# yumingj/C2-Matching

Measured on AMD Instinct MI355X. Metric: LR-Ref image pairs/sec (160x160 LR, 500x500 Ref, 4x SR), higher is better.
Workload: dtype f32

## Files before the change

### c2-matching_amd/c2m_amd/ops.py

```python
import torch

from . import _lib


def _dev_f32(t, name):
    if not isinstance(t, torch.Tensor) or not t.is_cuda:
        raise _lib.C2MError(f"{name} must be a tensor on the GPU (the HIP path has no CPU fallback)")
    if t.dtype != torch.float32:
        raise _lib.C2MError(f"{name} must be float32, got {t.dtype}")
    return t if t.is_contiguous() else t.contiguous()


def _stream():
    return torch.cuda.current_stream().cuda_stream


def _pair(v):
    return (int(v), int(v)) if isinstance(v, int) else (int(v[0]), int(v[1]))


class NormalizedFeatures(torch.Tensor):

    @staticmethod
    def wrap(t, ss):
# ... 589 lines not shown


def _wino4_ok(srcs, weight, out_mode, W):
    return _WINO4 and W % 64 == 0 and out_mode == "nhwc" and _wino_ok(srcs, weight, out_mode, W)


def bf16_autocast():
    return torch.is_autocast_enabled('cuda') and torch.get_autocast_dtype('cuda') == torch.bfloat16


def _split_ok(srcs, weight, fast):
    return ((_SPLIT == "all" or (fast and _SPLIT != "0")) and all(s.shape[1] % 16 == 0 for s in srcs) and
            sum(s.shape[1] for s in srcs) == weight.shape[1])


def conv3x3(srcs, weight, bias=None, act=ACT_NONE, slope=0.1, res1=None, res2=None, out_mode="nhwc", out=None, algo=None,
            out2_grouped8=None, fast=False, out_dtype=None, dword_stores=False):
    srcs = list(srcs) if isinstance(srcs, (list, tuple)) else [srcs]
    B, _, H, W = srcs[0].shape
    Cin = sum(s.shape[1] for s in srcs)
    Cout = weight.shape[0]
    dev = srcs[0].device
    if algo is None:
        reduced = bf16_autocast()
        if (out2_grouped8 is None and (_split_ok(srcs, weight, fast) or (reduced and _split_ok(srcs, weight, True))) and (out_mode != "nhwc_pool2" or (H % 2 == 0 and W % 2 == 0))
                and (out_mode not in ("nhwc", "nhwc_pool2") or Cout % 4 == 0)):
            kind = 4 if reduced else 6 if _f16x2_auto() else 3
        else:
            kind = 2 if (fast and _wino4_ok(srcs, weight, out_mode, W)) else 1 if _wino_ok(srcs, weight, out_mode, W) else 0
    elif algo in ALGO_IDS:
        kind = ALGO_IDS[algo]
    else:
        raise _lib.C2MError(f"conv3x3: unknown algo {algo!r} (one of {', '.join(ALGO_IDS)})")
# ... 15 lines not shown
    if out is not None:
        out_dtype = out.dtype
    if out_dtype == torch.bfloat16:
        io |= 2
    elif out_dtype not in (None, torch.float32):
        raise _lib.C2MError("conv3x3: out_dtype is float32 or bfloat16")
    for bit, r in ((4, res1), (8, res2)):
        if r is not None and r.dtype == torch.bfloat16:
            io |= bit
    if io and (kind != 4 or out_mode != "nhwc"):
        raise _lib.C2MError("conv3x3: bfloat16 tensors need the bf16 kernel (algo='bf16' / bf16 autocast) in nhwc mode")
    if dword_stores:
        if io or kind not in (3, 4, 6) or out_mode not in ("pixel_shuffle", "nchw"):
            raise _lib.C2MError("conv3x3: dword_stores selects a store path of the split kernels' pixel_shuffle / nchw epilogues")
        io = 16
    d.io_flags = io
    d.wr = wr.data_ptr()
    if bias is not None:
        bias = _dev_f32(bias.detach(), "bias")
    d.bias = bias.data_ptr() if bias is not None else None
    d.act, d.slope = int(act), float(slope)
    if out_mode == "nhwc":
        if out is None:
            out = empty_nhwc(B, Cout, H, W, dev, torch.bfloat16 if io & 2 else torch.float32)
        d.out_mode = 0
        o = _nhwc_src(out, "out", bf16_ok=True)
        d.out_pix_pitch, d.out_row_pitch, d.out_img_pitch = o.pix_pitch, o.row_pitch, o.img_pitch
        for name, r in (("res1", res1), ("res2", res2)):
            if r is not None:
                rs = _nhwc_src(r, name, bf16_ok=True)
# ... 15 lines not shown
        o = _nhwc_src(out, "out")
        d.out_pix_pitch, d.out_row_pitch, d.out_img_pitch = o.pix_pitch, o.row_pitch, o.img_pitch
    elif out_mode == "nchw":
        out = torch.empty((B, Cout, H, W), dtype=torch.float32, device=dev)
        d.out_mode = 2
    else:
        raise _lib.C2MError(f"unknown out_mode {out_mode}")
    d.out = out.data_ptr()
    if kind == 6:
        d.range_flag = _range_flag(dev).data_ptr()
    with torch.cuda.device(dev):
        _lib.check(_lib.lib().c2m_conv3x3_nhwc_f32(_stream(), d), "c2m_conv3x3_nhwc_f32")
    if _ConvFlops.enabled:
        f = 2.0 * Cout * 9 * Cin * H * W * B
        _ConvFlops.add(_KINDS[kind].family, f, f * _KINDS[kind].exec_factor)
    return out


def conv3x3_dgrad(grad_out, weight):
    Cout, Cin = weight.shape[:2]
    B, Cg, H, W = grad_out.shape
    if Cg != Cout or Cout % 16 != 0 or Cin % 4 != 0:
        raise _lib.C2MError("conv3x3_dgrad: grad_out channels must equal weight.shape[0] (a multiple of 16); Cin % 4 == 0")
    wr = _wcache.get(weight, kind=5)
    out = empty_nhwc(B, Cin, H, W, grad_out.device)
    d = _lib.Conv3x3Desc()
    d.algo = _KINDS[5].algo
    d.B, d.H, d.W, d.Cin, d.Cout, d.nsrc = B, H, W, Cout, Cin, 1
    d.src[0] = _nhwc_src(grad_out, "grad_out")
    d.wr = wr.data_ptr()
    d.out_mode = 0
# ... 127 lines not shown


def index_to_flow(max_idx):
    if not max_idx.is_cuda or max_idx.dtype != torch.int64 or max_idx.dim() != 3:
        raise _lib.C2MError("max_idx must be an int64 GPU tensor [B, hq, wq]")
    mi = max_idx.contiguous()
    B, hq, wq = mi.shape
    flow = torch.empty((B, hq, wq, 2), dtype=torch.float32, device=mi.device)
    with torch.cuda.device(mi.device):
        _lib.check(_lib.lib().c2m_index_to_flow_f32(_stream(), mi.data_ptr(), B, hq, wq, flow.data_ptr()), "c2m_index_to_flow_f32")
    return flow


def conv3x3_dcn_head(srcs, weight, bias, deformable_groups, flow=None, scale=1, abs_sum=None, algo=None):
    srcs = list(srcs) if isinstance(srcs, (list, tuple)) else [srcs]
    B, _, H, W = srcs[0].shape
    Cin = sum(s.shape[1] for s in srcs)
    dg = int(deformable_groups)
    Cout = weight.shape[0]
    if Cout != 3 * dg * 9:
        raise _lib.C2MError("conv3x3_dcn_head: weight must have 3*dg*9 output channels")
    dev = srcs[0].device
    bias = _dev_f32(bias.detach(), "bias")
    offset = torch.empty((B, 2 * dg * 9, H, W), dtype=torch.float32, device=dev)
    mask = torch.empty((B, dg * 9, H, W), dtype=torch.float32, device=dev)
    if flow is not None:
        if flow.dtype != torch.float32 or not flow.is_cuda or flow.dim() != 4 or flow.shape[0] != B or flow.shape[3] != 2:
            raise _lib.C2MError("flow must be float32 [B, fh, fw, 2] on the GPU")
        flow = flow.contiguous()
    if abs_sum is not None and (abs_sum.dtype != torch.float64 or abs_sum.numel() < 256 or not abs_sum.is_cuda):
        raise _lib.C2MError("abs_sum must be a float64 GPU tensor with 256 slots (C2M_ABS_SUM_SLOTS)")
    split = (Cout // 64) * 64
    slices = [(0, Cout)] if (split == 0 or Cout - split > 32 or split == Cout) else [(0, split), (split, Cout)]
    use_split = algo in ("split", "bf16", "split16") or (algo is None and _SPLIT != "0" and all(s_.shape[1] % 16 == 0 for s_ in srcs))
    split_id = (4 if (algo == "bf16" or (algo is None and bf16_autocast())) else
                6 if (algo == "split16" or (algo is None and _f16x2_auto())) else 3)
    fam = []
    for (c0, c1) in slices:
        kind = split_id if use_split else int(_WINO and algo is None and (c1 - c0) % 64 == 0 and W % 32 == 0 and
                                       all(s_.shape[1] % 16 == 0 for s_ in srcs))
        fam.append(kind)
        wr = _wcache.get(weight, rows=(c0, c1), kind=kind)
        d = _lib.Conv3x3Desc()
        d.algo = _KINDS[kind].algo
        d.B, d.H, d.W, d.Cin, d.Cout, d.nsrc = B, H, W, Cin, c1 - c0, len(srcs)
        for k, s in enumerate(srcs):
            d.src[k] = _nhwc_src(s, f"src{k}")
        d.wr = wr.data_ptr()
        d.bias = bias.data_ptr() + 4 * c0
        d.out_mode = 3
        d.out, d.mask_out, d.n_off, d.scale = offset.data_ptr(), mask.data_ptr(), 2 * dg * 9, int(scale)
        d.cout_offset, d.cout_total = c0, Cout
        if flow is not None:
            d.flow, d.fh, d.fw = flow.data_ptr(), flow.shape[1], flow.shape[2]
        if abs_sum is not None:
            d.abs_sum = abs_sum.data_ptr()
        if kind == 6:
            d.range_flag = _range_flag(dev).data_ptr()
        with torch.cuda.device(dev), _apply_switch("head"):
            _lib.check(_lib.lib().c2m_conv3x3_nhwc_f32(_stream(), d), "c2m_conv3x3_nhwc_f32")
    if _ConvFlops.enabled:
        for (c0, c1), k in zip(slices, fam):
            f = 2.0 * (c1 - c0) * 9 * Cin * H * W * B
            _ConvFlops.add("dcn_head_" + _KINDS[k].family, f, f * _KINDS[k].exec_factor)
    return offset, mask


class BorderedNHWC:
    grouped8 = None

    def __new__(cls, x=None):
        pre = bordered_of(x) if x is not None else None
        return pre if pre is not None else super().__new__(cls)
# ... 345 lines not shown
```

### c2-matching_amd/csrc/conv3x3.hip

```cpp
#include <stdio.h>
#include <stdlib.h>

#include <type_traits>

#include "c2m_common.h"
#include "conv3x3_shared.h"

namespace c2m {
namespace conv {

constexpr int TW = 32, TH = 4;
constexpr int HW_ = TW + 2, HH_ = TH + 2;
constexpr int NPIX = HW_ * HH_;
constexpr int KCH = 32;
constexpr int NIN_REAL = (NPIX * 8 + 63) / 64;
constexpr int NIN_W = 7;
constexpr int IN_BYTES = NIN_REAL * 1024;
static_assert(NIN_REAL <= 4 * NIN_W, "four waves x NIN_W instructions must cover the halo tile");

__global__ void __launch_bounds__(256) conv3x3_relayout_kernel(const float* __restrict__ w, int Cin, int Cout, int MW,
                                                                 long long total, float* __restrict__ wr) {
  const long long e0 = (long long)blockIdx.x * 256 + threadIdx.x;
  if (e0 >= total + 64) return;
  if (e0 >= total) { wr[e0] = 0.0f; return; }
// ... 1371 lines not shown
  p.out_pix_pitch = d->out_pix_pitch; p.out_row_pitch = d->out_row_pitch; p.out_img_pitch = d->out_img_pitch;
  p.res1 = d->res1; p.res2 = d->res2; p.mask_out = d->mask_out; p.flow = d->flow; p.fh = d->fh; p.fw = d->fw;
  p.scale = d->scale; p.n_off = d->n_off; p.abs_sum = d->abs_sum;
  p.scale_shift = -1;
  for (int sh = 0; sh < 16; ++sh)
    if (d->scale == (1 << sh)) p.scale_shift = sh;
  if (d->out_mode == 3 && d->flow && p.scale_shift < 0) return C2M_ERR_UNSUPPORTED;
  if (d->out_mode == 3 && (long long)std::max(d->n_off, cout_total - d->n_off) * d->H * d->W * 4 >= 0x7fffffffLL) return C2M_ERR_UNSUPPORTED;
  p.out_vec4 = out_vec4 ? 1 : 0;
  p.co_off = d->out_mode == 3 ? d->cout_offset : 0;
  p.cout_total = cout_total;
  p.out2 = d->out2; p.out2_row_pitch = d->out2_row_pitch; p.out2_plane_pitch = d->out2_plane_pitch;
  p.out2_img_pitch = d->out2_img_pitch;
  p.range_flag = d->range_flag;
  p.io_flags = d->io_flags;
  if (d->io_flags & C2M_IO_DWORD_STORES) {
    if (!splitk || (d->out_mode != 1 && d->out_mode != 2) || (d->io_flags & ~C2M_IO_DWORD_STORES)) return C2M_ERR_UNSUPPORTED;
  } else if (d->io_flags != 0) {
    if (d->algo != C2M_CONV_BF16 || d->out_mode != 0 || (d->io_flags & ~15)) return C2M_ERR_UNSUPPORTED;
    if ((d->io_flags & C2M_IO_SRC_BF16) && (d->nsrc != 1 || d->src[0].pix_pitch % 8 != 0 || d->src[0].row_pitch % 8 != 0 || d->src[0].img_pitch % 8 != 0))
      return C2M_ERR_UNSUPPORTED;
    if (d->Cout % ((d->io_flags & C2M_IO_OUT_BF16) ? 8 : 4) != 0) return C2M_ERR_UNSUPPORTED;
    if ((d->io_flags & C2M_IO_OUT_BF16) && (d->out_pix_pitch % 8 != 0 || d->out_row_pitch % 8 != 0 || d->out_img_pitch % 8 != 0)) return C2M_ERR_UNSUPPORTED;
  }
  if (d->out2 && (wino || d->out_mode != 0 || !out_vec4 || d->Cout % 8 != 0 || ((uintptr_t)d->out2 & 15) ||
                  d->out2_row_pitch % 4 != 0 || d->out2_plane_pitch % 4 != 0 || d->out2_img_pitch % 4 != 0))
    return C2M_ERR_UNSUPPORTED;

  const int MW = wino ? 64 : conv_mw(d->Cout);
  const long long ntile = (long long)p.tiles_x * p.tiles_y * p.B;
  if ((wino || splitk) && (d->out_mode == 0 || d->out_mode == 4) && !out_vec4) return C2M_ERR_UNSUPPORTED;
// ... 86 lines not shown
```

### c2-matching_amd/csrc/conv3x3_split.hip

```cpp
#include <stdio.h>
#include <stdlib.h>

#include <algorithm>
#include <type_traits>

#include "c2m_common.h"
#include "conv3x3_shared.h"

namespace c2m {
namespace conv {
namespace split {

typedef __bf16 bf16x8 __attribute__((ext_vector_type(8)));
typedef unsigned u32x2 __attribute__((ext_vector_type(2)));

constexpr int KC = 16;
constexpr int TWX = 32, THY = 8;
constexpr int HWc = TWX + 2, HHr = THY + 2;
constexpr int NPIX = HWc * HHr;
constexpr int NRAW_W = (NPIX * 4 + 255) / 256;
constexpr int NRAW = 4 * NRAW_W;
constexpr int RAW_BYTES = NRAW * 1024;
constexpr int HALFB = NPIX * 16;
static_assert(HALFB % 128 == 64 && HALFB % 16 == 0, "bank phase of the second k half");
// ... 161 lines not shown
  r[3] = 0x00020000;
  return r;
}
template <int IMM>
__device__ __forceinline__ void buf_load128(bf16x8& d, unsigned voff, const i32x4 rsrc, int soff) {
  asm volatile("buffer_load_dwordx4 %0, %1, %2, %3 offen offset:%4" : "=v"(d) : "v"(voff), "s"(rsrc), "s"(soff), "n"(IMM) : "memory");
}
__device__ __forceinline__ void buf_load128f(f32x4& d, unsigned voff, const i32x4 rsrc, int soff) {
  asm volatile("buffer_load_dwordx4 %0, %1, %2, %3 offen" : "=v"(d) : "v"(voff), "s"(rsrc), "s"(soff) : "memory");
}
template <int IMM>
__device__ __forceinline__ void lds_write64(unsigned addr, const u32x2 v) {
  asm volatile("ds_write_b64 %0, %1 offset:%2" ::"v"(addr), "v"(v), "n"(IMM) : "memory");
}

template <int FL, int MT, int MODE, int ABL = 0, bool IO16 = false>
__global__ void __launch_bounds__(256, 2) conv3x3_split_kernel(Params p) {
  static_assert(!IO16 || (FL == 1 && MODE == 0 && (ABL & 4) == 0), "bf16 sources: the bf16 flavour's channels-last mode");
  constexpr int NT = 2;
  constexpr int MW = 32 * MT;
  using PR = Flavour<FL>;
  constexpr int NPX = PR::NPX, NPW = PR::NPW;
  constexpr int PLB = IO16 ? 12 * 1024 : NPX * 2 * HALFB;
  constexpr bool PIPE = FL != 3;
#ifndef C2M_SPLIT_BF
#define C2M_SPLIT_BF 1
#endif
  constexpr bool BFA = ABL == 0 && C2M_SPLIT_BF != 0;
  constexpr bool BF = BFA && !IO16;
  constexpr bool BF16S = BFA && IO16;
  constexpr int NPB = IO16 ? 3 : (PIPE ? 2 : 1);
  constexpr int NRING = PIPE ? 3 : 2;
  constexpr int WTAP = NPW * MT * 1024;
  constexpr int WUNIT = 3 * WTAP;
  constexpr int NWI = WUNIT / 1024;
  constexpr int NW_W = (NWI + 3) / 4;
  extern __shared__ __attribute__((aligned(1024))) char lds[];
  const unsigned lds0 = (unsigned)(uintptr_t)(__attribute__((address_space(3))) char*)lds;
  const unsigned pl_base = lds0, w_base = lds0 + NPB * PLB, dummy = w_base + NRING * WUNIT, bias_lds = dummy + 1024;

  const int tid = threadIdx.x, l = tid & 63, hi = l >> 5, j = l & 31;
  const int wv = __builtin_amdgcn_readfirstlane(tid >> 6);
  const int ntile = p.tiles_x * p.tiles_y * p.B;
  const int tile_first = xcd_remap(blockIdx.x, gridDim.x) * p.tpw;
// ... 54 lines not shown
    }
  };
  auto set_source = [&](const Src& S) __attribute__((always_inline)) {
#pragma unroll
    for (int sl = 0; sl < NRAW_W; ++sl) {
      const int c = slotc[sl];
      const int iy = iy0 - 1 + (c & 0xff), ix = ix0 - 1 + ((c >> 8) & 0xff);
      const unsigned bad = ((c >> 24) != 0 && (unsigned)iy < (unsigned)p.H && (unsigned)ix < (unsigned)p.W) ? 0u : 1u;
      ivoff[sl] = ((unsigned)(iy * S.row_pitch + ix * S.pix_pitch + 4 * ((c >> 16) & 3)) * 4u) | (bad << 31);
    }
  };
  auto src_rsrc = [&](const Src& S, int b) __attribute__((always_inline)) {
    const unsigned bytes = (unsigned)((p.H - 1) * S.row_pitch + (p.W - 1) * S.pix_pitch + S.C) * 4u;
    return make_rsrc_words(S.ptr + (long long)b * S.img_pitch, bytes);
  };
  int in_soff = 0;
  bool in_first = true;
  auto issue_in_begin = [&]() __attribute__((always_inline)) {
    const int c0 = dma_c * KC;
    in_first = c0 < p.src[0].C;
    if (++dma_c == p.nchunks) dma_c = 0;
    if constexpr (IO16) {
      if (c0 == 0) {
        ib = dma_tc.b; iy0 = dma_tc.ty * THY; ix0 = dma_tc.tx * TWX;
        tc_next(dma_tc);
        const Src& S = p.src[0];
        in_rs16 = make_rsrc(reinterpret_cast<const char*>(S.ptr) + (long long)ib * S.img_pitch * 2,
                            (unsigned)((p.H - 1) * S.row_pitch + (p.W - 1) * S.pix_pitch + S.C) * 2u);
        set_source16(S);
      }
      in_soff = c0 * 2;
      return;
    }
    if (c0 == 0) {
      ib = dma_tc.b; iy0 = dma_tc.ty * THY; ix0 = dma_tc.tx * TWX;
      tc_next(dma_tc);
      rs0 = src_rsrc(p.src[0], ib);
      rs1 = src_rsrc(p.src[1], ib);
      set_source(p.src[0]);
    } else if (c0 == p.src[0].C) {
      set_source(p.src[1]);
    }
    in_soff = (in_first ? c0 : c0 - p.src[0].C) * 4;
  };
  __amdgpu_buffer_rsrc_t in_rs16_cur = in_rs16;
  const __amdgpu_buffer_rsrc_t null_rs16 = make_rsrc(p.src[0].ptr, 0u);
  auto issue_in_dma = [&](int sl, unsigned plane_off) __attribute__((always_inline)) {
    __builtin_amdgcn_raw_ptr_buffer_load_lds(BF16S ? in_rs16_cur : in_rs16, (__attribute__((address_space(3))) void*)(pl_base + plane_off + (unsigned)(wv + 4 * sl) * 1024u), 16,
                                             dvoff[sl], in_soff, 0, 0);
  };
  f32x4 rawr[NRAW_W];
  i32x4 rs_cur = {0, 0, 0, 0x00020000};
  auto set_chunk_rsrc = [&](bool live) __attribute__((always_inline)) {
    const i32x4 r = in_first ? rs0 : rs1;
    rs_cur[0] = r[0];
    rs_cur[1] = r[1];
    rs_cur[2] = live ? r[2] : 0;
    rs_cur[3] = 0x00020000;
  };
  auto issue_in_piece = [&](auto slc) __attribute__((always_inline)) {
    constexpr int sl = decltype(slc)::value;
    if constexpr (BF) {
      buf_load128f(rawr[sl], ivoff[sl], rs_cur, in_soff);
    } else {
// ... 67 lines not shown
      if (trace_it >= 0) {
        unsigned long long t;
        asm volatile("s_memtime %0\n\ts_waitcnt lgkmcnt(0)" : "=s"(t)::"memory");
        const unsigned tl = (unsigned)t;
        const int ln = trace_it * 26 + ev;
        trace_v = l == ln ? tl : trace_v;
      }
    }
  };

  issue_in_begin();
  if constexpr (IO16) {
    in_rs16_cur = in_rs16;
#pragma unroll
    for (int sl = 0; sl < 3; ++sl) issue_in_dma(sl, 0u);
  } else {
    if constexpr (BF) set_chunk_rsrc(true);
    static_for<0, NRAW_W>([&](auto rr) __attribute__((always_inline)) { issue_in_piece(rr); });
  }
#pragma unroll
  for (int i = 0; i < NW_W; ++i) issue_w_piece(0u, i);
  issue_w_done();
  if constexpr (NRING == 3) {
    if (3 * G > 1) {
#pragma unroll
      for (int i = 0; i < NW_W; ++i) issue_w_piece((unsigned)WUNIT, i);
      issue_w_done();
    }
  }
  if constexpr (IO16) {
    if (G > 1) {
      issue_in_begin();
      in_rs16_cur = in_rs16;
#pragma unroll
      for (int sl = 0; sl < 3; ++sl) issue_in_dma(sl, (unsigned)PLB);
    }
    wait_vmcnt<0>();
    asm volatile("s_waitcnt lgkmcnt(0)" ::: "memory");
    __builtin_amdgcn_s_barrier();
  }
  wait_vmcnt<0>();
  if constexpr (PIPE && !IO16) {
    const bool more1 = !(ABL & 2) && G > 1;
    if (more1) issue_in_begin();
    if constexpr (BF) set_chunk_rsrc(more1);
    static_for<0, NRAW_W>([&](auto rr) __attribute__((always_inline)) {
      constexpr int R = decltype(rr)::value;
      conv_split(rawr[R]);
      conv_store(rr, cdst);
      if (more1) issue_in_piece(rr);
    });
    asm volatile("s_waitcnt lgkmcnt(0)" ::: "memory");
    __builtin_amdgcn_s_barrier();
  }

  constexpr int NG = PR::N;
#ifndef C2M_LPGD
#define C2M_LPGD 2
#endif
  constexpr int LPGD = C2M_LPGD;
  constexpr int LPG = NG >= 4 ? (NLA + NLB + NG - 3) / (NG - 2) : (NG == 3 ? (NLA + NLB + LPGD - 1) / LPGD : NLA + NLB);
  static_assert(NRAW_W == 6, "two split rounds per unit");
  unsigned slot_cur = 0u;
  for (int it = 0, gc = 0; it < ntl; ++it) {
    if constexpr ((ABL & 1024) != 0) trace_it = (it >= p.co_off && it < p.co_off + 2 && p.nchunks <= 4) ? it - p.co_off : -1;
    for (int c = 0; c < p.nchunks; ++c, ++gc) {
      const bool has_next = PIPE ? gc + 1 < G : true;
      const bool more_in = !(ABL & 2) && gc + (PIPE ? 2 : 1) < G;
      const unsigned pb = IO16 ? (unsigned)(gc % 3) * PLB : PIPE ? (unsigned)(gc & 1) * PLB : 0u;
      const unsigned pb_in = (unsigned)((gc + 2) % 3) * PLB;
      const unsigned bcur = bbase + pb, cnext = PIPE ? cdst + (PLB - pb) : cdst;
      if (more_in) issue_in_begin();
      if constexpr (BF) set_chunk_rsrc(more_in);
      if constexpr (BF16S) in_rs16_cur = more_in ? in_rs16 : null_rs16;
      if constexpr (!PIPE) {
        if constexpr (!(ABL & 4)) {
          static_for<0, NRAW_W>([&](auto rr) __attribute__((always_inline)) {
            constexpr int R = decltype(rr)::value;
            conv_split(rawr[R]);
            conv_store(rr, cdst);
            if (BF || more_in) issue_in_piece(rr);
          });
        }
        asm volatile("s_waitcnt lgkmcnt(0)" ::: "memory");
        __builtin_amdgcn_s_barrier();
      }
      static_for<0, 3>([&](auto dyc) __attribute__((always_inline)) {
        constexpr int dy = decltype(dyc)::value;
        const int u = 3 * gc + dy;
// ... 27 lines not shown
                           std::integral_constant<int, K - NLA>(), bcur);
                }
              });
            }
            if constexpr (dx == 0) {
              if constexpr (BFA) {
#pragma unroll
                for (int i = g; i < NW_W; i += NG) issue_w_piece(slot_nxt, i, do_w);
              } else {
                if (do_w) {
#pragma unroll
                  for (int i = g; i < NW_W; i += NG) issue_w_piece(slot_nxt, i);
                }
              }
            }
            if constexpr (FL == 2 && g == 0) {
#pragma unroll
              for (int mt = 0; mt < MT; ++mt) {
                const f16x8 sc = {(_Float16)(1.0f / F16_LO_SCALE), (_Float16)(1.0f / F16_LO_SCALE), (_Float16)(1.0f / F16_LO_SCALE), (_Float16)(1.0f / F16_LO_SCALE),
                                  (_Float16)(1.0f / F16_LO_SCALE), (_Float16)(1.0f / F16_LO_SCALE), (_Float16)(1.0f / F16_LO_SCALE), (_Float16)(1.0f / F16_LO_SCALE)};
                Ad[mt] = __builtin_bit_cast(bf16x8, __builtin_bit_cast(f16x8, A[set][0][mt]) * sc);
              }
            }
            if constexpr (IO16 && dx == 1 && g == NG / 2) {
              if (BF16S || more_in) issue_in_dma(dy, pb_in);
            }
            if constexpr (PIPE && !IO16 && dx >= 1 && g == NG / 2 && !(ABL & 4)) {
              constexpr int R = dx >= 1 ? 2 * dy + dx - 1 : 0;
              if (BF || has_next) {
                if constexpr (dy == 0) {
                  if (gc == 0) wait_vmcnt<0>();
                }
                conv_split(rawr[R]);
                conv_store(std::integral_constant<int, R>(), cnext);
                if (BF || more_in) issue_in_piece(std::integral_constant<int, R>());
              }
            }
            if constexpr (!(ABL & 16) && !((ABL & 256) && dx == 2)) {
#pragma unroll
              for (int mt = 0; mt < MT; ++mt)
#pragma unroll
                for (int nq = 0; nq < NT; ++nq) {
// ... 3 lines not shown
                    acc[mt][nt] = __builtin_amdgcn_mfma_f32_32x32x16_f16(__builtin_bit_cast(f16x8, av),
                                                                         __builtin_bit_cast(f16x8, Bq[set][PR::X[g]][nt]), acc[mt][nt], 0, 0, 0);
                  else
                    acc[mt][nt] = __builtin_amdgcn_mfma_f32_32x32x16_bf16(av, Bq[set][PR::X[g]][nt], acc[mt][nt], 0, 0, 0);
                }
            }
            __builtin_amdgcn_sched_barrier(0);
          });
          if constexpr (dx == 0) {
            if constexpr (BFA) issue_w_done(do_w);
            else if (do_w) issue_w_done();
          }
        });
        if (!(ABL & 8)) {
          asm volatile("s_waitcnt lgkmcnt(0)" ::: "memory");
          if constexpr (BF && PIPE) {
            wait_vmcnt<4 + NW_W>();
          } else if constexpr (BF16S) {
            wait_vmcnt<2 + NW_W>();
          } else if (IO16 && more_in) {
            wait_vmcnt<2 + NW_W>();
          } else if (PIPE && !IO16 && more_in) {
            if ((ABL & 128) && c == 0 && dy == 0) wait_vmcnt<4 + NW_W + 16>();
            else wait_vmcnt<4 + NW_W>();
          } else wait_vmcnt<0>();
          stamp(2 * (3 * c + dy));
          __builtin_amdgcn_s_barrier();
          stamp(2 * (3 * c + dy) + 1);
        }
        slot_cur = slot_cur == (unsigned)((NRING - 1) * WUNIT) ? 0u : slot_cur + (unsigned)WUNIT;
      });
// ... 26 lines not shown
    bf16x8r hres[NT][MT][2];
    if constexpr (EPI_FAST16) {
      fast16 = (p.io_flags & 6) == 6 && p.res1 != nullptr && cb * MW + MW <= p.Cout && y0 + THY <= p.H && x0 + TWX <= p.W;
      if (fast16) {
        const __bf16* rb = reinterpret_cast<const __bf16*>(p.res1) + (size_t)b * p.out_img_pitch + (size_t)(y0 + 2 * wv) * p.out_row_pitch +
                           (size_t)(x0 + j) * p.out_pix_pitch + cb * MW + 8 * hi;
#pragma unroll
        for (int nt = 0; nt < NT; ++nt)
#pragma unroll
          for (int mt = 0; mt < MT; ++mt)
#pragma unroll
            for (int k = 0; k < 2; ++k) hres[nt][mt][k] = *reinterpret_cast<const bf16x8r*>(rb + (size_t)nt * p.out_row_pitch + mt * 32 + 16 * k);
      }
    }
    if constexpr (EPI_FAST) {
      fast = p.out_vec4 != 0 && cb * MW + MW <= p.Cout && y0 + THY <= p.H && x0 + TWX <= p.W && (FL != 1 || (p.io_flags & 14) == 0);
      fpix = (size_t)b * p.out_img_pitch + (size_t)(y0 + 2 * wv) * p.out_row_pitch + (size_t)(x0 + j) * p.out_pix_pitch + co_e;
      if (fast && p.res1 != nullptr) res_load(p.res1, 0);
    }
#pragma unroll
    for (int mt = 0; mt < MT; ++mt)
#pragma unroll
      for (int qd = 0; qd < 4; ++qd) {
        const f32x4 bv = *(const __attribute__((address_space(3))) f32x4*)(bias_lds + (mt * 32 + 8 * qd + 4 * hi) * 4);
#pragma unroll
        for (int nt = 0; nt < NT; ++nt)
#pragma unroll
          for (int e = 0; e < 4; ++e) {
            if constexpr (FL == 2) acc[mt][nt][4 * qd + e] = acc[mt][nt][4 * qd + e] * w_sinv + bv[e];
            else acc[mt][nt][4 * qd + e] += bv[e];
          }
// ... 63 lines not shown
        const int yo = (y0 >> 1) + wv, xo = (x0 + j) >> 1;
        const bool pok = (y0 + 2 * wv + 1) < p.H && (x0 + j) < p.W && (j & 1) == 0;
        float* ob = p.out + (size_t)b * p.out_img_pitch + (size_t)yo * p.out_row_pitch + (size_t)xo * p.out_pix_pitch + co_e;
#pragma unroll
        for (int mt = 0; mt < MT; ++mt)
#pragma unroll
          for (int qd = 0; qd < 4; ++qd) {
            f32x4 v;
#pragma unroll
            for (int e = 0; e < 4; ++e) {
              const float m = fmaxf(acc[mt][0][4 * qd + e], acc[mt][1][4 * qd + e]);
              v[e] = fmaxf(m, __shfl_xor(m, 1, 64));
            }
            if (pok && co_e + mt * 32 + 8 * qd + 3 < p.Cout) *reinterpret_cast<f32x4*>(ob + mt * 32 + 8 * qd) = v;
          }
      } else if (EPI_FAST && fast) {
        static_assert(NT == 2, "two pixel rows per wave");
        auto store_row = [&](int nt) __attribute__((always_inline)) {
#pragma unroll
          for (int mt = 0; mt < MT; ++mt)
#pragma unroll
            for (int qd = 0; qd < 4; ++qd) {
              f32x4 v;
#pragma unroll
              for (int e = 0; e < 4; ++e) v[e] = acc[mt][nt][4 * qd + e];
              *reinterpret_cast<f32x4*>(p.out + fpix + (size_t)nt * p.out_row_pitch + mt * 32 + 8 * qd) = v;
            }
        };
        if (p.res1 != nullptr) { res_add(0); res_load(p.res1, 1); }
        if (p.res2 != nullptr) {
// ... 251 lines not shown
        switch (abl) {
          case 0: break;
          case 1: go16(&split::conv3x3_split_kernel<1, 2, 0, 1, true>, dn[0]); return rc;
          case 2: go16(&split::conv3x3_split_kernel<1, 2, 0, 2, true>, dn[1]); return rc;
          case 8: go16(&split::conv3x3_split_kernel<1, 2, 0, 8, true>, dn[2]); return rc;
          case 16: go16(&split::conv3x3_split_kernel<1, 2, 0, 16, true>, dn[3]); return rc;
          case 32: go16(&split::conv3x3_split_kernel<1, 2, 0, 32, true>, dn[4]); return rc;
          case 64: go16(&split::conv3x3_split_kernel<1, 2, 0, 64, true>, dn[5]); return rc;
          case 43: go16(&split::conv3x3_split_kernel<1, 2, 0, 43, true>, dn[6]); return rc;
          case 48: go16(&split::conv3x3_split_kernel<1, 2, 0, 48, true>, dn[7]); return rc;
          case 107: go16(&split::conv3x3_split_kernel<1, 2, 0, 107, true>, dn[8]); return rc;
          default: fprintf(stderr, "c2m: unknown C2M_SPLIT_ABL16 mask\n"); return C2M_ERR_INVALID_ARG;
        }
      }
      go16(&split::conv3x3_split_kernel<1, MT, 0, 0, true>, done16);
      return rc;
    }
  }
  if constexpr (NP == 2 && MT == 2) {
    static const int abl = [] {
      const char* e = getenv("C2M_SPLIT_ABL");
      const int v = e ? atoi(e) : 0;
      if (v > 0) fprintf(stderr, "c2m: C2M_SPLIT_ABL=%d -- conv3x3 split kernel runs a timing-only ablation, its results are wrong\n", v);
      return v;
    }();
    static unsigned long long done_abl[13] = {};
    if (abl > 0 && p.out_mode == 0) {
      switch (abl) {
        case 1: go(&split::conv3x3_split_kernel<NP, 2, 0, 1>, done_abl[1]); break;
        case 2: go(&split::conv3x3_split_kernel<NP, 2, 0, 2>, done_abl[2]); break;
// ... 98 lines not shown
```

### c2-matching_amd/mmsr/models/archs/ref_restoration_arch.py

```python
import torch
import torch.nn as nn
import torch.nn.functional as F

import mmsr.models.archs.arch_util as arch_util
from c2m_amd import ops as _ops
from mmsr.models.archs.DCNv2.dcn_v2 import DCN_sep_pre_multi_offset as DynAgg
from mmsr.models.archs.DCNv2.dcn_v2 import FusedPreOffset, use_conv_kernels


class ContentExtractor(nn.Module):

    def __init__(self, in_nc=3, out_nc=3, nf=64, n_blocks=16):
        super(ContentExtractor, self).__init__()
        self.conv_first = nn.Conv2d(in_nc, nf, 3, 1, 1)
        self.body = arch_util.make_layer(arch_util.ResidualBlockNoBN, n_blocks, nf=nf)
        self.lrelu = nn.LeakyReLU(negative_slope=0.1, inplace=True)
        arch_util.default_init_weights([self.conv_first], 0.1)

    def forward(self, x):
        return self.body(self.lrelu(self.conv_first(x)))

    def forward_train(self, x):
        f = self.lrelu(self.conv_first(x)).contiguous(memory_format=torch.channels_last)
        return _train_body(self.body, f)
# ... 42 lines not shown
        t = _conv_t(blk.conv1, [f], _ops.ACT_RELU)
        f = _conv_t(blk.conv2, [t]) + f
    return f if skip is None else f + skip


def _fused_body(body, f, skip=None):
    n = len(body)
    if _BF16_IO and _ops._SPLIT != "0" and _ops.bf16_autocast() and blk_bf16_ok(body):
        bf = torch.bfloat16
        for k, blk in enumerate(body):
            t = _ops.conv3x3(f, blk.conv1.weight, blk.conv1.bias, act=_ops.ACT_RELU, fast=True, out_dtype=bf)
            f = _ops.conv3x3(t, blk.conv2.weight, blk.conv2.bias, res1=f, res2=skip if k == n - 1 else None, fast=True,
                             out_dtype=None if k == n - 1 else bf)
        return f
    for k, blk in enumerate(body):
        t = _ops.conv3x3(f, blk.conv1.weight, blk.conv1.bias, act=_ops.ACT_RELU, fast=True)
        f = _ops.conv3x3(t, blk.conv2.weight, blk.conv2.bias, res1=f, res2=skip if k == n - 1 else None, fast=True)
    return f


_BF16_IO = _os.environ.get("C2M_BF16_IO", "1") != "0"


def blk_bf16_ok(body):
    return all(b.conv1.weight.shape[0] % 16 == 0 and b.conv1.weight.shape[1] % 16 == 0 and b.conv2.weight.shape[0] % 16 == 0 for b in body)


class DynamicAggregationRestoration(nn.Module):

    _STAGES = (('small', 'relu3_1', 256), ('medium', 'relu2_1', 128), ('large', 'relu1_1', 64))

# ... 151 lines not shown
```

### include/c2m_hip.h

```cpp
#ifndef C2M_HIP_H
#define C2M_HIP_H

#include <stddef.h>
#include <stdint.h>

#ifdef __cplusplus
extern "C" {
#endif

typedef void* c2m_stream_t;

typedef enum c2m_status {
  C2M_OK = 0,
  C2M_ERR_INVALID_ARG = 1,
  C2M_ERR_UNSUPPORTED = 2,
  C2M_ERR_WORKSPACE = 3,
  C2M_ERR_LAUNCH = 4,
  C2M_ERR_NO_DEVICE = 5
} c2m_status;

int c2m_abi_version(void);
const char* c2m_status_string(int status);
const char* c2m_last_hip_error(void);
int c2m_device_arch(char* buf, int buflen);
// ... 110 lines not shown
  double* abs_sum;
  int algo;
  int cout_offset;
  int cout_total;
  float* out2;
  int out2_row_pitch;
  long long out2_plane_pitch, out2_img_pitch;
  int* range_flag;
  int io_flags;
} c2m_conv3x3_desc;
#define C2M_IO_SRC_BF16 1
#define C2M_IO_OUT_BF16 2
#define C2M_IO_RES1_BF16 4
#define C2M_IO_RES2_BF16 8
#define C2M_IO_DWORD_STORES 16

size_t c2m_conv3x3_relayout_bytes(int Cin, int Cout);
int c2m_conv3x3_relayout_f32(c2m_stream_t stream, const float* weight , int Cin, int Cout, float* wr);
size_t c2m_conv3x3_relayout_wino_bytes(int Cin, int Cout);
int c2m_conv3x3_relayout_wino_f32(c2m_stream_t stream, const float* weight, int Cin, int Cout, float* wr);
size_t c2m_conv3x3_relayout_wino4_bytes(int Cin, int Cout);
int c2m_conv3x3_relayout_wino4_f32(c2m_stream_t stream, const float* weight, int Cin, int Cout, float* wr);
size_t c2m_conv3x3_relayout_split_bytes(int Cin, int Cout, int pieces);
int c2m_conv3x3_relayout_split_f32(c2m_stream_t stream, const float* weight, int Cin, int Cout, int pieces, void* wr);
int c2m_conv3x3_relayout_split_multi(c2m_stream_t stream, const long long* jobs, int njobs, long long nblocks, int any_f16);
int c2m_conv3x3_nhwc_f32(c2m_stream_t stream, const c2m_conv3x3_desc* desc);

int c2m_conv3x3_relayout_split_dgrad_f32(c2m_stream_t stream, const float* weight , int Cin, int Cout,
                                         int pieces, void* wr);
size_t c2m_conv3x3_wgrad_workspace_bytes(int B, int H, int W, int Cin, int Cout);
// ... 30 lines not shown
```

Measured before the change: 116.0.

## Hand off conv1 output to conv2 as pre-split f16x2 pieces in residual blocks

Adds a path where the first conv of each residual block writes its output already split into two f16 pieces in a planar piece layout. The second conv then loads those pieces straight into LDS with buffer-load-to-LDS, skipping its own fp32 load and f16x2 split of the activation. This is meant to cut the conversion work and register pressure in the consumer's input pipeline, at the cost of a new epilogue with permlane swaps, different wait counts and more kernel variants. It is gated to inference with no bf16 autocast and no stream capture, and only when the f16x2 kernel is auto-selected.

```diff
diff --git a/c2-matching_amd/c2m_amd/ops.py b/c2-matching_amd/c2m_amd/ops.py
--- a/c2-matching_amd/c2m_amd/ops.py
+++ b/c2-matching_amd/c2m_amd/ops.py
@@ -627,9 +627,38 @@
             sum(s.shape[1] for s in srcs) == weight.shape[1])
 
 
+_SPLIT_HANDOFF = _os.environ.get("C2M_SPLIT_HANDOFF", "1") != "0"
+
+
+class F16x2Pieces:
+
+    __slots__ = ("buf",)
+
+    def __init__(self, buf):
+        self.buf = buf
+
+    @property
+    def shape(self):
+        return self.buf.shape
+
+    @property
+    def device(self):
+        return self.buf.device
+
+
+def split_handoff_ok(src, weight):
+    return (_SPLIT_HANDOFF and not torch.is_grad_enabled() and not bf16_autocast() and weight.shape[0] % 16 == 0 and
+            _split_ok([src], weight, True) and not torch.cuda.is_current_stream_capturing() and _f16x2_auto())
+
+
 def conv3x3(srcs, weight, bias=None, act=ACT_NONE, slope=0.1, res1=None, res2=None, out_mode="nhwc", out=None, algo=None,
-            out2_grouped8=None, fast=False, out_dtype=None, dword_stores=False):
+            out2_grouped8=None, fast=False, out_dtype=None, dword_stores=False, out_pieces=False):
     srcs = list(srcs) if isinstance(srcs, (list, tuple)) else [srcs]
+    pieces_in = isinstance(srcs[0], F16x2Pieces)
+    if any(isinstance(s, F16x2Pieces) for s in srcs[1:]) or (pieces_in and len(srcs) != 1):
+        raise _lib.C2MError("conv3x3: an F16x2Pieces source must be the only source")
+    if pieces_in:
+        srcs = [srcs[0].buf]
     B, _, H, W = srcs[0].shape
     Cin = sum(s.shape[1] for s in srcs)
     Cout = weight.shape[0]
@@ -675,6 +704,11 @@
         if io or kind not in (3, 4, 6) or out_mode not in ("pixel_shuffle", "nchw"):
             raise _lib.C2MError("conv3x3: dword_stores selects a store path of the split kernels' pixel_shuffle / nchw epilogues")
         io = 16
+    if pieces_in or out_pieces:
+        if kind != 6 or io or out2_grouped8 is not None or (out_pieces and (out_mode != "nhwc" or out is not None or Cout % 16 != 0)):
+            raise _lib.C2MError("conv3x3: f16 x 2 pieces need the f16 x 2 kernel (algo='split16' / a guarded forward), fp32 "
+                                "tensors otherwise, and out_pieces 'nhwc' mode with Cout % 16 == 0")
+        io = (32 if pieces_in else 0) | (64 if out_pieces else 0)
     d.io_flags = io
     d.wr = wr.data_ptr()
     if bias is not None:
@@ -720,7 +754,7 @@
     if _ConvFlops.enabled:
         f = 2.0 * Cout * 9 * Cin * H * W * B
         _ConvFlops.add(_KINDS[kind].family, f, f * _KINDS[kind].exec_factor)
-    return out
+    return F16x2Pieces(out) if out_pieces else out
 
 
 def conv3x3_dgrad(grad_out, weight):
@@ -878,6 +912,11 @@
 
 def conv3x3_dcn_head(srcs, weight, bias, deformable_groups, flow=None, scale=1, abs_sum=None, algo=None):
     srcs = list(srcs) if isinstance(srcs, (list, tuple)) else [srcs]
+    pieces_in = isinstance(srcs[0], F16x2Pieces)
+    if any(isinstance(s, F16x2Pieces) for s in srcs[1:]) or (pieces_in and len(srcs) != 1):
+        raise _lib.C2MError("conv3x3_dcn_head: an F16x2Pieces source must be the only source")
+    if pieces_in:
+        srcs = [srcs[0].buf]
     B, _, H, W = srcs[0].shape
     Cin = sum(s.shape[1] for s in srcs)
     dg = int(deformable_groups)
@@ -903,6 +942,8 @@
     for (c0, c1) in slices:
         kind = split_id if use_split else int(_WINO and algo is None and (c1 - c0) % 64 == 0 and W % 32 == 0 and
                                        all(s_.shape[1] % 16 == 0 for s_ in srcs))
+        if pieces_in and (kind != 6 or W % 4 != 0):
+            raise _lib.C2MError("conv3x3_dcn_head: f16 x 2 pieces need the f16 x 2 kernel and W % 4 == 0")
         fam.append(kind)
         wr = _wcache.get(weight, rows=(c0, c1), kind=kind)
         d = _lib.Conv3x3Desc()
@@ -921,6 +962,7 @@
             d.abs_sum = abs_sum.data_ptr()
         if kind == 6:
             d.range_flag = _range_flag(dev).data_ptr()
+        d.io_flags = 32 if pieces_in else 0
         with torch.cuda.device(dev), _apply_switch("head"):
             _lib.check(_lib.lib().c2m_conv3x3_nhwc_f32(_stream(), d), "c2m_conv3x3_nhwc_f32")
     if _ConvFlops.enabled:
diff --git a/c2-matching_amd/csrc/conv3x3.hip b/c2-matching_amd/csrc/conv3x3.hip
--- a/c2-matching_amd/csrc/conv3x3.hip
+++ b/c2-matching_amd/csrc/conv3x3.hip
@@ -1409,7 +1409,19 @@
   p.out2_img_pitch = d->out2_img_pitch;
   p.range_flag = d->range_flag;
   p.io_flags = d->io_flags;
-  if (d->io_flags & C2M_IO_DWORD_STORES) {
+  if (d->io_flags & (C2M_IO_SRC_F16X2 | C2M_IO_OUT_F16X2)) {
+    constexpr int pieces = C2M_IO_SRC_F16X2 | C2M_IO_OUT_F16X2;
+    if (d->algo != C2M_CONV_SPLIT_F16X2 || (d->io_flags & ~pieces)) return C2M_ERR_INVALID_ARG;
+    const long long hw = (long long)d->H * d->W;
+    if ((d->io_flags & C2M_IO_SRC_F16X2) &&
+        (d->nsrc != 1 || (d->out_mode != 0 && d->out_mode != 3) || d->src[0].pix_pitch != d->Cin ||
+         (long long)d->src[0].row_pitch != (long long)d->W * d->Cin || d->src[0].img_pitch != hw * d->Cin || hw * d->Cin * 4 >= 0x7fffffffLL))
+      return C2M_ERR_INVALID_ARG;
+    if ((d->io_flags & C2M_IO_OUT_F16X2) &&
+        (d->out_mode != 0 || d->Cout % 16 != 0 || d->out_pix_pitch != d->Cout || (long long)d->out_row_pitch != (long long)d->W * d->Cout ||
+         d->out_img_pitch != hw * d->Cout || hw * d->Cout * 4 >= 0x7fffffffLL))
+      return C2M_ERR_INVALID_ARG;
+  } else if (d->io_flags & C2M_IO_DWORD_STORES) {
     if (!splitk || (d->out_mode != 1 && d->out_mode != 2) || (d->io_flags & ~C2M_IO_DWORD_STORES)) return C2M_ERR_UNSUPPORTED;
   } else if (d->io_flags != 0) {
     if (d->algo != C2M_CONV_BF16 || d->out_mode != 0 || (d->io_flags & ~15)) return C2M_ERR_UNSUPPORTED;
diff --git a/c2-matching_amd/csrc/conv3x3_split.hip b/c2-matching_amd/csrc/conv3x3_split.hip
--- a/c2-matching_amd/csrc/conv3x3_split.hip
+++ b/c2-matching_amd/csrc/conv3x3_split.hip
@@ -199,9 +199,10 @@
   asm volatile("ds_write_b64 %0, %1 offset:%2" ::"v"(addr), "v"(v), "n"(IMM) : "memory");
 }
 
-template <int FL, int MT, int MODE, int ABL = 0, bool IO16 = false>
+template <int FL, int MT, int MODE, int ABL = 0, bool IO16 = false, bool PSRC = false>
 __global__ void __launch_bounds__(256, 2) conv3x3_split_kernel(Params p) {
   static_assert(!IO16 || (FL == 1 && MODE == 0 && (ABL & 4) == 0), "bf16 sources: the bf16 flavour's channels-last mode");
+  static_assert(!PSRC || (FL == 2 && (MODE == 0 || MODE == 5) && ABL == 0 && !IO16), "f16 x 2 piece sources: f16 x 2, modes 0 / 5");
   constexpr int NT = 2;
   constexpr int MW = 32 * MT;
   using PR = Flavour<FL>;
@@ -212,7 +213,7 @@
 #define C2M_SPLIT_BF 1
 #endif
   constexpr bool BFA = ABL == 0 && C2M_SPLIT_BF != 0;
-  constexpr bool BF = BFA && !IO16;
+  constexpr bool BF = BFA && !IO16 && !PSRC;
   constexpr bool BF16S = BFA && IO16;
   constexpr int NPB = IO16 ? 3 : (PIPE ? 2 : 1);
   constexpr int NRING = PIPE ? 3 : 2;
@@ -297,12 +298,37 @@
     const unsigned bytes = (unsigned)((p.H - 1) * S.row_pitch + (p.W - 1) * S.pix_pitch + S.C) * 4u;
     return make_rsrc_words(S.ptr + (long long)b * S.img_pitch, bytes);
   };
+  constexpr int PS_N = (4 * NPIX + 63) / 64;
+  unsigned psoff[NRAW_W];
+  __amdgpu_buffer_rsrc_t ps_rs = make_rsrc(p.src[0].ptr, 0u);
+  auto set_source_ps = [&]() __attribute__((always_inline)) {
+    const int hw = p.H * p.W;
+#pragma unroll
+    for (int sl = 0; sl < NRAW_W; ++sl) {
+      const int q = min(64 * (wv + 4 * sl), 4 * NPIX - 64) + l, s = q / NPIX, pix = q - s * NPIX;
+      const int ry = pix / HWc, rx = pix - ry * HWc;
+      const int iy = iy0 - 1 + ry, ix = ix0 - 1 + rx;
+      const unsigned bad = ((unsigned)iy < (unsigned)p.H && (unsigned)ix < (unsigned)p.W) ? 0u : 1u;
+      psoff[sl] = ((unsigned)(s * hw + iy * p.W + ix) * 16u) | (bad << 31);
+    }
+  };
   int in_soff = 0;
   bool in_first = true;
   auto issue_in_begin = [&]() __attribute__((always_inline)) {
     const int c0 = dma_c * KC;
     in_first = c0 < p.src[0].C;
     if (++dma_c == p.nchunks) dma_c = 0;
+    if constexpr (PSRC) {
+      if (c0 == 0) {
+        ib = dma_tc.b; iy0 = dma_tc.ty * THY; ix0 = dma_tc.tx * TWX;
+        tc_next(dma_tc);
+        const unsigned img = (unsigned)p.Cin * (unsigned)(p.H * p.W) * 4u;
+        ps_rs = make_rsrc(reinterpret_cast<const char*>(p.src[0].ptr) + (size_t)ib * img, img);
+        set_source_ps();
+      }
+      in_soff = (c0 / KC) * 64 * p.H * p.W;
+      return;
+    }
     if constexpr (IO16) {
       if (c0 == 0) {
         ib = dma_tc.b; iy0 = dma_tc.ty * THY; ix0 = dma_tc.tx * TWX;
@@ -331,6 +357,12 @@
   auto issue_in_dma = [&](int sl, unsigned plane_off) __attribute__((always_inline)) {
     __builtin_amdgcn_raw_ptr_buffer_load_lds(BF16S ? in_rs16_cur : in_rs16, (__attribute__((address_space(3))) void*)(pl_base + plane_off + (unsigned)(wv + 4 * sl) * 1024u), 16,
                                              dvoff[sl], in_soff, 0, 0);
+  };
+  __amdgpu_buffer_rsrc_t ps_rs_cur = ps_rs;
+  auto issue_ps_piece = [&](int sl, unsigned plane_off) __attribute__((always_inline)) {
+    const int n = wv + 4 * sl;
+    const unsigned dst = n < PS_N ? pl_base + plane_off + (unsigned)min(64 * n, 4 * NPIX - 64) * 16u : dummy;
+    __builtin_amdgcn_raw_ptr_buffer_load_lds(ps_rs_cur, (__attribute__((address_space(3))) void*)dst, 16, psoff[sl], in_soff, 0, 0);
   };
   f32x4 rawr[NRAW_W];
   i32x4 rs_cur = {0, 0, 0, 0x00020000};
@@ -428,6 +460,10 @@
     in_rs16_cur = in_rs16;
 #pragma unroll
     for (int sl = 0; sl < 3; ++sl) issue_in_dma(sl, 0u);
+  } else if constexpr (PSRC) {
+    ps_rs_cur = ps_rs;
+#pragma unroll
+    for (int sl = 0; sl < NRAW_W; ++sl) issue_ps_piece(sl, 0u);
   } else {
     if constexpr (BF) set_chunk_rsrc(true);
     static_for<0, NRAW_W>([&](auto rr) __attribute__((always_inline)) { issue_in_piece(rr); });
@@ -454,7 +490,10 @@
     __builtin_amdgcn_s_barrier();
   }
   wait_vmcnt<0>();
-  if constexpr (PIPE && !IO16) {
+  if constexpr (PSRC) {
+    asm volatile("s_waitcnt lgkmcnt(0)" ::: "memory");
+    __builtin_amdgcn_s_barrier();
+  } else if constexpr (PIPE && !IO16) {
     const bool more1 = !(ABL & 2) && G > 1;
     if (more1) issue_in_begin();
     if constexpr (BF) set_chunk_rsrc(more1);
@@ -480,13 +519,14 @@
     if constexpr ((ABL & 1024) != 0) trace_it = (it >= p.co_off && it < p.co_off + 2 && p.nchunks <= 4) ? it - p.co_off : -1;
     for (int c = 0; c < p.nchunks; ++c, ++gc) {
       const bool has_next = PIPE ? gc + 1 < G : true;
-      const bool more_in = !(ABL & 2) && gc + (PIPE ? 2 : 1) < G;
+      const bool more_in = !(ABL & 2) && gc + (PIPE && !PSRC ? 2 : 1) < G;
       const unsigned pb = IO16 ? (unsigned)(gc % 3) * PLB : PIPE ? (unsigned)(gc & 1) * PLB : 0u;
       const unsigned pb_in = (unsigned)((gc + 2) % 3) * PLB;
       const unsigned bcur = bbase + pb, cnext = PIPE ? cdst + (PLB - pb) : cdst;
       if (more_in) issue_in_begin();
       if constexpr (BF) set_chunk_rsrc(more_in);
       if constexpr (BF16S) in_rs16_cur = more_in ? in_rs16 : null_rs16;
+      if constexpr (PSRC) ps_rs_cur = more_in ? ps_rs : null_rs16;
       if constexpr (!PIPE) {
         if constexpr (!(ABL & 4)) {
           static_for<0, NRAW_W>([&](auto rr) __attribute__((always_inline)) {
@@ -544,6 +584,9 @@
                 }
               }
             }
+            if constexpr (PSRC && dy < 2 && g == NG - 1) {
+              issue_ps_piece(3 * dy + dx, (unsigned)PLB - pb);
+            }
             if constexpr (FL == 2 && g == 0) {
 #pragma unroll
               for (int mt = 0; mt < MT; ++mt) {
@@ -555,7 +598,7 @@
             if constexpr (IO16 && dx == 1 && g == NG / 2) {
               if (BF16S || more_in) issue_in_dma(dy, pb_in);
             }
-            if constexpr (PIPE && !IO16 && dx >= 1 && g == NG / 2 && !(ABL & 4)) {
+            if constexpr (PIPE && !IO16 && !PSRC && dx >= 1 && g == NG / 2 && !(ABL & 4)) {
               constexpr int R = dx >= 1 ? 2 * dy + dx - 1 : 0;
               if (BF || has_next) {
                 if constexpr (dy == 0) {
@@ -589,7 +632,9 @@
         });
         if (!(ABL & 8)) {
           asm volatile("s_waitcnt lgkmcnt(0)" ::: "memory");
-          if constexpr (BF && PIPE) {
+          if constexpr (PSRC) {
+            wait_vmcnt<dy == 0 ? NW_W + 3 : (dy == 1 ? NW_W + 6 : NW_W)>();
+          } else if constexpr (BF && PIPE) {
             wait_vmcnt<4 + NW_W>();
           } else if constexpr (BF16S) {
             wait_vmcnt<2 + NW_W>();
@@ -646,7 +691,8 @@
       }
     }
     if constexpr (EPI_FAST) {
-      fast = p.out_vec4 != 0 && cb * MW + MW <= p.Cout && y0 + THY <= p.H && x0 + TWX <= p.W && (FL != 1 || (p.io_flags & 14) == 0);
+      fast = p.out_vec4 != 0 && cb * MW + MW <= p.Cout && y0 + THY <= p.H && x0 + TWX <= p.W && (FL != 1 || (p.io_flags & 14) == 0) &&
+             (FL != 2 || (p.io_flags & C2M_IO_OUT_F16X2) == 0);
       fpix = (size_t)b * p.out_img_pitch + (size_t)(y0 + 2 * wv) * p.out_row_pitch + (size_t)(x0 + j) * p.out_pix_pitch + co_e;
       if (fast && p.res1 != nullptr) res_load(p.res1, 0);
     }
@@ -740,6 +786,45 @@
             }
             if (pok && co_e + mt * 32 + 8 * qd + 3 < p.Cout) *reinterpret_cast<f32x4*>(ob + mt * 32 + 8 * qd) = v;
           }
+      } else if (FL == 2 && MODE == 0 && (p.io_flags & C2M_IO_OUT_F16X2)) {
+        const int hw = p.H * p.W, x = x0 + j;
+#pragma unroll
+        for (int nt = 0; nt < NT; ++nt) {
+          const int y = y0 + 2 * wv + nt;
+          if (y >= p.H || x >= p.W) continue;
+          const size_t opix = (size_t)b * p.out_img_pitch + (size_t)y * p.out_row_pitch + (size_t)x * p.out_pix_pitch;
+          float* ob = p.out + (size_t)b * p.Cout * hw + ((size_t)hi * hw + (size_t)(y * p.W + x)) * 4;
+#pragma unroll
+          for (int mt = 0; mt < MT; ++mt)
+#pragma unroll
+            for (int k = 0; k < 2; ++k) {
+              f32x4 v0, v1;
+#pragma unroll
+              for (int e = 0; e < 4; ++e) {
+                const float lo = acc[mt][nt][8 * k + e], up = acc[mt][nt][8 * k + 4 + e];
+                const auto r = __builtin_amdgcn_permlane32_swap(__builtin_bit_cast(unsigned, lo), __builtin_bit_cast(unsigned, up), false, false);
+                const unsigned r0 = r[0], r1 = r[1];
+                v0[e] = __builtin_bit_cast(float, r0);
+                v1[e] = __builtin_bit_cast(float, r1);
+              }
+              const int co16 = cb * MW + mt * 32 + 16 * k;
+              if (co16 < p.Cout) {
+                const int co8 = co16 + 8 * hi;
+                if (p.res1) { v0 += *reinterpret_cast<const f32x4*>(p.res1 + opix + co8); v1 += *reinterpret_cast<const f32x4*>(p.res1 + opix + co8 + 4); }
+                if (p.res2) { v0 += *reinterpret_cast<const f32x4*>(p.res2 + opix + co8); v1 += *reinterpret_cast<const f32x4*>(p.res2 + opix + co8 + 4); }
+                u32x2 a0, a1, b0, b1;
+                split2_f16(v0, a0, a1);
+                split2_f16(v1, b0, b1);
+                asm volatile("v_max3_f32 %0, %0, |%1|, |%2|\n\tv_max3_f32 %0, %0, |%3|, |%4|"
+                             : "+v"(amax) : "v"(v0[0]), "v"(v0[1]), "v"(v0[2]), "v"(v0[3]));
+                asm volatile("v_max3_f32 %0, %0, |%1|, |%2|\n\tv_max3_f32 %0, %0, |%3|, |%4|"
+                             : "+v"(amax) : "v"(v1[0]), "v"(v1[1]), "v"(v1[2]), "v"(v1[3]));
+                float* o = ob + (size_t)(co16 / KC) * 16 * hw;
+                *reinterpret_cast<u32x4*>(o) = u32x4{a0[0], a0[1], b0[0], b0[1]};
+                *reinterpret_cast<u32x4*>(o + (size_t)8 * hw) = u32x4{a1[0], a1[1], b1[0], b1[1]};
+              }
+            }
+        }
       } else if (EPI_FAST && fast) {
         static_assert(NT == 2, "two pixel rows per wave");
         auto store_row = [&](int nt) __attribute__((always_inline)) {
@@ -1021,6 +1106,15 @@
         }
       }
       go16(&split::conv3x3_split_kernel<1, MT, 0, 0, true>, done16);
+      return rc;
+    }
+  }
+  if constexpr (NP == 2) {
+    if (p.io_flags & C2M_IO_SRC_F16X2) {
+      static unsigned long long dps[2] = {};
+      if (p.out_mode == 0) go(&split::conv3x3_split_kernel<2, MT, 0, 0, false, true>, dps[0]);
+      else if (p.out_mode == 3 && p.W % 4 == 0 && g_head_stores != 0) go(&split::conv3x3_split_kernel<2, MT, 5, 0, false, true>, dps[1]);
+      else rc = C2M_ERR_UNSUPPORTED;
       return rc;
     }
   }
diff --git a/c2-matching_amd/mmsr/models/archs/ref_restoration_arch.py b/c2-matching_amd/mmsr/models/archs/ref_restoration_arch.py
--- a/c2-matching_amd/mmsr/models/archs/ref_restoration_arch.py
+++ b/c2-matching_amd/mmsr/models/archs/ref_restoration_arch.py
@@ -80,7 +80,8 @@
                              out_dtype=None if k == n - 1 else bf)
         return f
     for k, blk in enumerate(body):
-        t = _ops.conv3x3(f, blk.conv1.weight, blk.conv1.bias, act=_ops.ACT_RELU, fast=True)
+        pieces = _ops.split_handoff_ok(f, blk.conv1.weight) and blk.conv2.weight.shape[1] == blk.conv1.weight.shape[0]
+        t = _ops.conv3x3(f, blk.conv1.weight, blk.conv1.bias, act=_ops.ACT_RELU, fast=True, out_pieces=pieces)
         f = _ops.conv3x3(t, blk.conv2.weight, blk.conv2.bias, res1=f, res2=skip if k == n - 1 else None, fast=True)
     return f
 
diff --git a/include/c2m_hip.h b/include/c2m_hip.h
--- a/include/c2m_hip.h
+++ b/include/c2m_hip.h
@@ -148,6 +148,8 @@
 #define C2M_IO_RES1_BF16 4
 #define C2M_IO_RES2_BF16 8
 #define C2M_IO_DWORD_STORES 16
+#define C2M_IO_SRC_F16X2 32
+#define C2M_IO_OUT_F16X2 64
 
 size_t c2m_conv3x3_relayout_bytes(int Cin, int Cout);
 int c2m_conv3x3_relayout_f32(c2m_stream_t stream, const float* weight , int Cin, int Cout, float* wr);
```

Result: faster. 117.5 (median of 6 runs) (+1.3%).
